# brianz98/A-Fortran-Electronic-Structure-Program

Measured on AMD Instinct MI355X. Metric: CCSD iter wall-time (s) + (T) wall-time (s); fp64 TFLOP/s vs MFMA peak, higher is better.
Workload: dtype f64; 1 GPU; cfg5: nocc=20 nvirt=200, synthetic hashed ERIs scale 0.005; step = 1 CCSD iteration (replicated) + full (T) over i<=j<=k sharded across ranks; nocc=20, nvirt=200, triples=1540, parallelism=(T) ijk-shard x1, CCSD replicas

## Files before the change

### a-fortran-electronic-structure-program_amd/csrc/afesp_internal.h

```cpp
#pragma once
#include <hip/hip_runtime.h>
#include <stdint.h>

#include <map>
#include <stdexcept>
#include <string>
#include <thread>
#include <vector>

#include "gett.h"
#include "tgemm.h"

namespace afesp {

struct Error : std::runtime_error {
    int code;
    Error(int c, const std::string& m) : std::runtime_error(m), code(c) {}
};

#define AFESP_HIP(expr)                                                                                    \
    do {                                                                                                   \
        hipError_t e_ = (expr);                                                                            \
        if (e_ != hipSuccess)                                                                              \
            throw ::afesp::Error(2, std::string(#expr) + ": " + hipGetErrorString(e_) + " (" + __FILE__ + \
// ... 121 lines not shown
    int64_t lam_clock = 0;
    const void* lt_ops_owner = nullptr;
    int64_t lt_ops_stamp = -1, lt_ops_scratch = -1;
    Tensor tensor(std::initializer_list<int64_t> dims);
    void sync();
    void quiesce();
    ~Context();
};

Tensor view(double* d, std::initializer_list<int64_t> dims);

void contract(Context& cx, double alpha, const Tensor& A, const char* la, const Tensor& B, const char* lb, double beta,
              const Tensor& C, const char* lc, int nbatch = 1, const int64_t* bA = nullptr, const int64_t* bB = nullptr,
              const int64_t* bC = nullptr, int force_split = 0, int force_tm = 0, int force_tn = 0);

struct ContractCall {
    double alpha;
    const Tensor* A;
    const char* la;
    const Tensor* B;
    const char* lb;
    double beta;
    const Tensor* C;
    const char* lc;
};
void contract_pair(Context& cx, const ContractCall& c1, const ContractCall& c2);

void permute_add(Context& cx, double alpha, const Tensor& in, const char* li, double beta, const Tensor& out,
                 const char* lo);

void k_fill(Context& cx, double* x, int64_t n, double val);
void k_copy(Context& cx, double* dst, const double* src, int64_t n);
void k_axpby(Context& cx, double* y, double a, const double* x, double b, int64_t n);
void k_ivv_diag(Context& cx, double* ivv, const double* y, const double* x, int o, int v, int a0, int a1);
void k_div(Context& cx, double* out, const double* num, const double* den, int64_t n);
void k_antisym_pair(Context& cx, double* out, const double* in, int64_t d0, int64_t d1, int64_t d2, int64_t d3,
                    int which);
void k_asym_c(Context& cx, double* asym, double* c, const double* t1, const double* t2, int o, int v);
void k_t2_update(Context& cx, double* t2, const double* r2, const double* r2b, const double* r2c, const double* v_oovv, const double* D2,
                 const double* pp, int o, int v, double* t1, const double* r1, const double* r1b, const double* D1, const double* r2y = nullptr);
void k_add_swapped(Context& cx, double* out, const double* y, int o, int v);
void k_r2_full(Context& cx, double* out, const double* r2, const double* pp, int o, int v);
void k_denominators(Context& cx, double* D1, double* D2, const double* e, int o, int v);
void k_vvvv_sympack_packed(Context& cx, double* vs, double* va, const double* packed, int o, int v, int64_t ks, int64_t ka);
void k_c_sympack(Context& cx, double* cs, double* ca, const double* c, int o, int v, int64_t ns, int64_t na, bool half = false);
void k_oooo_pair_expand_add(Context& cx, double* I, const double* xs, const double* xa, int o, int64_t ns, int64_t na);
void k_oooo_sympack(Context& cx, double* is, double* ia, const double* I, int o, int64_t ns, int64_t na);
void k_rows_append(Context& cx, double* dst, int64_t ld, int64_t k0, const double* src, int64_t ns, int64_t ncol);
void k_pp_expand(Context& cx, double* pp, const double* ps, const double* pa, int o, int v, int64_t ns, int64_t na,
                 int64_t p0 = 0, int64_t p1 = -1);
void k_vvx_sympack(Context& cx, double* ws, double* wa, const double* x, int v, int64_t ncol, int64_t ks, int64_t ka);
void k_pair_expand_add(Context& cx, double* out, const double* ps, const double* pa, int o, int64_t ncol, int64_t ns, int64_t na);
void k_ooov_r1_trace(Context& cx, double* r1x, const double* ps, const double* pa, int o, int v, int64_t ns, int64_t na);
void k_cc_energy(Context& cx, double* out2, const double* v_oovv, const double* t1, const double* t2, double* t2_old,
                 int o, int v);
void k_final_sum(Context& cx, double* out, int nq, bool accumulate);
void k_lincomb(Context& cx, double* out, const double* xbase, int64_t xstride, const double* coef_dev, int nx,
               int64_t n);
void k_diis_solve(Context& cx, double* coef, double* bmat, double* flag, int n, int nerr, int slot);
void k_diis_push(Context& cx, double* ht, double* he, const double* amp, const double* amp_s, const double* hist_e, int64_t stride, int ny,
                 int slot, int64_t n);
struct CCTail {
    double *t2, *t1;
    const double *r2, *r1, *voovv, *D2, *D1, *pp;
    double* t2_old;
    int o, v;
// ... 30 lines not shown
```

### a-fortran-electronic-structure-program_amd/csrc/ccsd.h

```cpp
#pragma once
#include "afesp_internal.h"

namespace afesp {

struct DiisRing {
    int nerr = 0, nact = 0, it = 0;
    int64_t nvec = 0;
    double *amp = nullptr;
    double *amp_s = nullptr;
    double *hist_t = nullptr, *hist_e = nullptr;
    double *coef = nullptr;
    double *bmat = nullptr;
    bool tail_pending = false;
    int tail_slot = 0, tail_n = 0;
    double tail_b[256];
};
void diis_alloc(Context& cx, DiisRing& r, int diis_nerr);
void diis_save(Context& cx, DiisRing& r);
void diis_update(Context& cx, DiisRing& r);

struct CCState : DiisRing {
    int o = 0, v = 0;
    bool ready = false;
    double* e = nullptr;
// ... 6 lines not shown
    int sh_rank = 0, sh_world = 1;
    int64_t* pp_tab = nullptr;
    bool pp_sym = false;
    double *pp_vs = nullptr, *pp_va = nullptr, *pp_cs = nullptr, *pp_ca = nullptr, *pp_ps = nullptr, *pp_pa = nullptr;
    int64_t pp_ks = 0, pp_ka = 0, pp_ns = 0, pp_na = 0, pp_kn = 0;
    int64_t pp_lds = 0, pp_lda = 0;
    double *pp_ts = nullptr, *pp_ta = nullptr;
    double *oo_vs = nullptr, *oo_va = nullptr;
    double *oo_xs = nullptr, *oo_xa = nullptr;
    bool cs_packed = false;
    double* r1x = nullptr;
    bool r1x_valid = false;
    int hist_plain = 0;
    bool amps_touched = true;
    int64_t pp_nm = 0;
    double *ov_ws = nullptr, *ov_wa = nullptr;
    Tensor I_vo, I_vv, I_oo_p, I_oo, c, asym, x_voov, I_oooo, I_ovov, I_voov, I_ooov_p;
    Tensor z_ooov;
    double energy = 0.0, energy_old = 0.0, rms = 0.0;
    void* tplan = nullptr;
    Tensor I_vovv_pp, I_ooov_pp;
    const double* eri_src = nullptr;
    double* eri_own = nullptr;
    bool have_cr = false;
    int64_t amp_epoch = 0, cr_epoch = 0;
    void* ring = nullptr;
    bool partials_live = false;
    int64_t frozen_id = 0;
};
void triples_plan_free(CCState& s);

bool ring_tg_applies(const CCState& s);
bool ring_tg_pack(Context& cx, CCState& s);
void ring_tg_intermediates(Context& cx, CCState& s);
void ring_tg_residual(Context& cx, CCState& s);
void ring_tg_materialize(Context& cx, CCState& s, const Tensor& I_ovov_out, const Tensor& I_voov_out);
bool ring_live(const CCState& s);
bool ring_res_live(const CCState& s);
void ring_res_clear(CCState& s);
void ring_invalidate(CCState& s);
void ring_reinit(CCState& s);
const double* ring_Y(const CCState& s);
void ring_free(Context& cx, CCState& s);

void ccsd_init(Context& cx, CCState& s, int o, int v, const double* eri_mo_dev, const double* e_host, int diis_nerr);
bool ccsd_can_reinit(const CCState& s, int o, int v, int diis_nerr);
void ccsd_need_vvvv(Context& cx, CCState& s);
void ccsd_refresh_sharding(Context& cx, CCState& s);
bool ccsd_uses_lanes(const CCState& s);
void ccsd_diis_save(Context& cx, CCState& s);
void ccsd_intermediates(Context& cx, CCState& s, bool save_for_diis = false);
void ccsd_amplitudes(Context& cx, CCState& s, bool defer_update = false);
void ccsd_tail_launch(Context& cx, CCState& s);
int ccsd_tail_read(Context& cx, CCState& s, double e_tol, double t_tol);
void ccsd_pp_ladder(Context& cx, CCState& s);
void ccsd_ooov_pair_form(Context& cx, CCState& s, double* out = nullptr, int64_t a0 = 0, int64_t a1 = 0);
const double* ccsd_residual_full(Context& cx, CCState& s, bool r2);
void ccsd_build_I_vovv_p(Context& cx, CCState& s, const Tensor& out);
bool pp_sym_pays(int64_t o, int64_t v);
int ccsd_energy(Context& cx, CCState& s, double e_tol, double t_tol);
void ccsd_energy_launch(Context& cx, CCState& s);
int ccsd_energy_read(Context& cx, CCState& s, double e_tol, double t_tol);
void ccsd_diis_update(Context& cx, CCState& s);
void ccsd_free(Context& cx, CCState& s);

int64_t triples_count(int o);
void triples_shard_bounds(int o, int v, bool cr, int world, int64_t* bounds);
int triples_block_size(int o, int v, bool cr);
// ... 6 lines not shown
```

### a-fortran-electronic-structure-program_amd/csrc/ccsd.hip

```cpp
#include <algorithm>
#include <cmath>
#include <cstdlib>
#include <cstring>

#include "ccsd.h"
#include "comm.h"
#include "fused.h"

namespace afesp {

static inline int64_t tri64(int64_t i, int64_t j) { return i >= j ? i * (i + 1) / 2 + j : j * (j + 1) / 2 + i; }

bool ccsd_can_reinit(const CCState& s, int o, int v, int diis_nerr)
{
    if (!knobs().cc_reinit) return false;
    return s.ready && s.o == o && s.v == v && s.nerr == diis_nerr && s.pp_sym == pp_sym_pays(o, v);
}

void ccsd_init(Context& cx, CCState& s, int o, int v, const double* eri_mo_dev, const double* e_host, int diis_nerr)
{
    if (o <= 0 || v <= 0) throw Error(1, "ccsd_init: need at least one occupied and one virtual orbital");
    const bool again = ccsd_can_reinit(s, o, v, diis_nerr);
    if (again) {
        cx.quiesce();
// ... 243 lines not shown
    } else {
        k_copy(cx, s.I_oo.d, s.I_oo_p.d, s.I_oo.size());
    }
    C(1.0, s.t1, "je", s.I_vo, "ei", 1.0, s.I_oo, "ji");
    lane(1);
    k_copy(cx, s.I_oooo.d, s.v_oooo.d, s.I_oooo.size());
    if (s.pp_sym && !par && !fused) ccsd_oooo_pair_form(cx, s);
    else C(1.0, s.c, "klef", s.v_oovv, "ijef", 1.0, s.I_oooo, "klij");
    C(1.0, s.t1, "ke", s.v_oovo, "ilej", 1.0, s.I_oooo, "klij");
    C(1.0, s.t1, "le", s.v_oovo, "jkei", 1.0, s.I_oooo, "klij");
    lane(2);
    const int64_t a_len = s.I_ovov.stride[3], a_off = v0 * a_len, a_cnt = (v1 - v0) * a_len;
    if (ivv_diag && s.sharded) {
        if (v1 > v0) C(1.0, s.t1, "je", sl(s.v_vvov, 3), "ebia", 0.0, sl(s.I_ovov, 3), "jbia");
    } else if (ivv_diag) {
        contract_pair(cx, {1.0, &s.t1, "je", &s.v_vvov, "ebia", 0.0, &s.I_ovov, "jbia"}, {1.0, &s.v_vvov, "beia", &s.t1, "je", 0.0, &s.x_voov, "bjia"});
    } else if (v1 > v0) {
        k_copy(cx, s.I_ovov.d + a_off, s.v_ovov.d + a_off, a_cnt);
        if (!ring) C(-0.5, s.v_oovv, "mibe", sl(s.c, 2), "mjae", 1.0, sl(s.I_ovov, 3), "jbia");
        C(-1.0, s.v_oovo, "mibj", sl(s.t1, 1), "ma", 1.0, sl(s.I_ovov, 3), "jbia");
        C(1.0, s.t1, "je", sl(s.v_vvov, 3), "ebia", 1.0, sl(s.I_ovov, 3), "jbia");
    }
    lane(3);
    if (s.sharded) { if (v1 > v0) C(1.0, sl(s.v_vvov, 3), "beia", s.t1, "je", 0.0, sl(s.x_voov, 3), "bjia"); }
    else if (!ivv_diag) C(1.0, s.v_vvov, "beia", s.t1, "je", 0.0, s.x_voov, "bjia");
    if (ivv_diag && v1 > v0) {
        k_ivv_diag(cx, s.I_vv.d, s.I_ovov.d, s.x_voov.d, s.o, s.v, (int)v0, (int)v1);
        k_axpby(cx, s.I_ovov.d + a_off, 1.0, s.v_ovov.d + a_off, 1.0, a_cnt);
        if (!ring) C(-0.5, s.v_oovv, "mibe", sl(s.c, 2), "mjae", 1.0, sl(s.I_ovov, 3), "jbia");
        C(-1.0, s.v_oovo, "mibj", sl(s.t1, 1), "ma", 1.0, sl(s.I_ovov, 3), "jbia");
    }
    const int x_voov_ready = par ? cx.mark() : 0;
    if (v1 > v0) {
        permute_add(cx, 1.0, sl(s.v_oovv, 2), "jiab", 0.0, sl(s.I_voov, 3), "bjia");
        if (fused) C(1.0, s.v_vvov, "beia", s.t1, "je", 1.0, s.I_voov, "bjia");
        else k_axpby(cx, s.I_voov.d + a_off, 1.0, s.x_voov.d + a_off, 1.0, a_cnt);
        if (!ring) {
            C(0.5, s.w_oovv, "imbe", sl(s.t2, 3), "mjea", 1.0, sl(s.I_voov, 3), "bjia");
            C(-0.5, s.v_oovv, "imbe", sl(s.c, 2), "mjae", 1.0, sl(s.I_voov, 3), "bjia");
        }
        C(-1.0, s.v_oovo, "imbj", sl(s.t1, 1), "ma", 1.0, sl(s.I_voov, 3), "bjia");
    }
    if (ring) ring_tg_intermediates(cx, s);
    lane(4);
    if (save_for_diis) diis_save(cx, s);
    if (fused) permute_add(cx, 1.0, s.v_oovo, "kjai", 0.0, s.z_ooov, "jkia");
    C(1.0, s.t1, "ie", s.v_oovv, "mjeb", fused ? 1.0 : 0.0, s.z_ooov, "ijmb");
    C(1.0, s.t1, "je", s.v_ovov, "mbie", 1.0, s.z_ooov, "ijmb");
    lane(5);
    permute_add(cx, 1.0, s.v_oovo, "kjai", 0.0, s.I_ooov_p, "jkia");
    if (s.sharded) {
        Tensor osh = view(cx.scratch("ooov_sh", s.I_ooov_p.size()), {(int64_t)s.o, (int64_t)s.o, (int64_t)s.o, (int64_t)s.v});
        if (v1 > v0) {
            if (s.pp_sym) {
                AFESP_HIP(hipMemsetAsync(osh.d + osh.stride[3] * v0, 0, sizeof(double) * osh.stride[3] * (v1 - v0), cx.stream));
                ccsd_ooov_pair_form(cx, s, osh.d, v0, v1);
            } else {
                C(1.0, s.t2, "jkef", sl(s.v_vvov, 3), "efia", 0.0, sl(osh, 3), "jkia");
            }
            if (par) cx.wait(x_voov_ready);
            C(1.0, s.t1, "je", sl(s.x_voov, 3), "ekia", 1.0, sl(osh, 3), "jkia");
        }
    } else if (s.pp_sym) {
        ccsd_ooov_pair_form(cx, s);
    } else {
        C(1.0, s.t2, "jkef", s.v_vvov, "efia", 1.0, s.I_ooov_p, "jkia");
    }
    if (par) cx.wait(x_voov_ready);
    if (!s.sharded) C(1.0, s.t1, "je", s.x_voov, "ekia", 1.0, s.I_ooov_p, "jkia");
// ... 225 lines not shown
        Tensor r1s = s.r1;
        r1s.d = s.r1_sh;
        C(1.0, s.t1, "ie", slice_axis(s.I_vv, 1, v0, v1), "ea", 1.0, slice_axis(r1s, 1, v0, v1), "ia");
        C(1.0, s.asym, "mief", sl(s.v_vvov, 3), "efma", 1.0, slice_axis(r1s, 1, v0, v1), "ia");
    }
    lane(3);
    if (!sh && !ring) C(1.0, s.asym, "miea", s.I_voov, "ejmb", par ? 0.0 : 1.0, r2c, "ijab");
    if (!open_with_vvov && !sh) C(1.0, s.t1, "ie", s.v_vvov, "baje", 1.0, r2c, "ijab");
    if (!sh) C(-1.0, s.t1, "ma", s.z_ooov, "ijmb", 1.0, r2c, "ijab");
    if (par) cx.join();
    if (sh) {
        const int64_t np = (int64_t)s.v * (s.v + 1) / 2;
        comm_allreduce_dev(cx, cx.comm, s.pp, (int64_t)s.o * s.o * np + s.r2.size() + s.r1.size());
        k_copy(cx, s.r2.d, s.r2_sh, s.r2.size());
        k_axpby(cx, s.r1.d, 1.0, s.r1_sh, 1.0, s.r1.size());
    }
    if (defer_update) return;
    k_t2_update(cx, s.t2.d, s.r2.d, par ? r2b.d : nullptr, par ? r2c.d : nullptr, s.v_oovv.d, s.D2.d, s.pp, s.o, s.v, s.t1.d, s.r1.d,
                par ? r1b.d : nullptr, s.D1.d, ring ? ring_Y(s) : nullptr);
}

const double* ccsd_residual_full(Context& cx, CCState& s, bool r2)
{
    const int64_t n = r2 ? s.r2.size() : s.r1.size();
    double* full = cx.scratch(r2 ? "r2_full" : "r1_full", n);
    auto add_partial = [&](const char* buf) {
        auto it = cx.cache.find(buf);
        if (s.partials_live && it != cx.cache.end()) k_axpby(cx, full, 1.0, (const double*)it->second.first, 1.0, n);
    };
    if (r2) {
        k_r2_full(cx, full, s.r2.d, s.pp, s.o, s.v);
        add_partial(R2_LANE2);
        add_partial(R2_LANE3);
        if (ring_res_live(s)) k_add_swapped(cx, full, ring_Y(s), s.o, s.v);
    } else {
        k_copy(cx, full, s.r1.d, n);
        add_partial(R1_LANE5);
    }
    return full;
}

void ccsd_build_I_vovv_p(Context& cx, CCState& s, const Tensor& out)
{
    permute_add(cx, 1.0, s.v_vvov, "baic", 0.0, out, "ciab");
    contract(cx, -1.0, s.v_oovv, "micb", s.t1, "ma", 1.0, out, "ciab");
    contract(cx, -1.0, s.v_ovov, "maic", s.t1, "mb", 1.0, out, "ciab");
}

void ccsd_tail_launch(Context& cx, CCState& s)
{
    auto launch = [](Context& c, CCState* st) {
        CCTail a;
        a.t2 = st->t2.d; a.t1 = st->t1.d; a.r2 = st->r2.d; a.r1 = st->r1.d; a.voovv = st->v_oovv.d; a.D2 = st->D2.d; a.D1 = st->D1.d;
        a.pp = st->pp; a.t2_old = st->t2_old.d; a.o = st->o; a.v = st->v;
        a.r2y = ring_res_live(*st) ? ring_Y(*st) : nullptr;
        a.half_hist = st->hist_plain == 0;
        if (st->hist_plain > 0) --st->hist_plain;
        a.nerr = st->nerr;
        a.ny = 0; a.slot = 0;
        a.ht = a.he = nullptr; a.amp_s = a.hist_e = nullptr; a.stride = st->nvec;
        a.coef = st->coef; a.bmat = st->bmat;
        if (st->nerr >= 2) {
            int it = st->it + 1;
            if (it > st->nerr) it -= st->nerr;
            a.slot = it - 1;
            a.ny = std::min(st->nact + 1, st->nerr);
            a.ht = st->hist_t + (int64_t)a.slot * st->nvec;
// ... 180 lines not shown
```

### a-fortran-electronic-structure-program_amd/csrc/kernels.hip

```cpp
#include "device_util.h"
#include "fused.h"

namespace afesp {

namespace {
__global__ void fill_kernel(double* x, int64_t n, double val) { GRID_STRIDE(i, n) x[i] = val; }
__global__ void axpby_kernel(double* y, double a, const double* x, double b, int64_t n)
{
    GRID_STRIDE(i, n) y[i] = a * x[i] + (b != 0.0 ? b * y[i] : 0.0);
}
__global__ void div_kernel(double* out, const double* num, const double* den, int64_t n) { GRID_STRIDE(i, n) out[i] = num[i] / den[i]; }

__global__ void antisym_pair_kernel(double* out, const double* in, int64_t d0, int64_t d1, int64_t d2, int64_t d3, int which)
{
    const int64_t n = d0 * d1 * d2 * d3;
    GRID_STRIDE(x, n)
    {
        int64_t i0 = x % d0, r = x / d0, i1 = r % d1;
        r /= d1;
        int64_t i2 = r % d2, i3 = r / d2;
        int64_t y = which == 0 ? i1 + d0 * (i0 + d1 * (i2 + d2 * i3)) : i0 + d0 * (i1 + d1 * (i3 + d2 * i2));
        out[x] = 2.0 * in[x] - in[y];
    }
}

__global__ void asym_c_kernel(double* asym, double* c, const double* t1, const double* t2, int o, int v)
{
    const int64_t n = (int64_t)o * o * v * v;
    GRID_STRIDE(x, n)
    {
        int i = (int)(x % o);
        int64_t r = x / o;
        int j = (int)(r % o);
        r /= o;
        int a = (int)(r % v), b = (int)(r / v);
        double t = t2[x];
        asym[x] = 2.0 * t - t2[j + (int64_t)o * (i + (int64_t)o * (a + (int64_t)v * b))];
        c[x] = t + t1[i + o * a] * t1[j + o * b];
    }
}

__global__ void t2_update_kernel(double* t2, const double* r2, const double* r2b, const double* r2c, const double* voovv, const double* D2,
                                 const double* pp, int o, int v, double* t1, const double* r1, const double* r1b, const double* D1,
                                 const double* r2y)
{
    const int64_t n = (int64_t)o * o * v * v, n1 = (int64_t)o * v;
    GRID_STRIDE(x, n)
    {
        int i = (int)(x % o);
        int64_t r = x / o;
        int j = (int)(r % o);
        r /= o;
        int a = (int)(r % v), b = (int)(r / v);
        int64_t y = j + (int64_t)o * (i + (int64_t)o * (b + (int64_t)v * a));
        const int64_t lad = (a <= b) ? i + (int64_t)o * (j + (int64_t)o * ((int64_t)b * (b + 1) / 2 + a))
                                     : j + (int64_t)o * (i + (int64_t)o * ((int64_t)a * (a + 1) / 2 + b));
        double rx = r2[x], ry = r2[y];
        if (r2b) { rx += r2b[x]; ry += r2b[y]; }
        if (r2c) { rx += r2c[x]; ry += r2c[y]; }
        if (r2y) {
            rx += r2y[j + (int64_t)o * (i + (int64_t)o * (a + (int64_t)v * b))];
            ry += r2y[i + (int64_t)o * (j + (int64_t)o * (b + (int64_t)v * a))];
        }
        t2[x] = (rx + ry + pp[lad] + voovv[x]) / D2[x];
        if (x < n1) t1[x] = (r1[x] + (r1b ? r1b[x] : 0.0)) / D1[x];
    }
}

__global__ void denominators_kernel(double* D1, double* D2, const double* e, int o, int v)
{
    const int64_t n = (int64_t)o * o * v * v;
    GRID_STRIDE(x, n)
    {
        int i = (int)(x % o);
        int64_t r = x / o;
        int j = (int)(r % o);
        r /= o;
        int a = (int)(r % v), b = (int)(r / v);
        D2[x] = e[i] + e[j] - e[a + o] - e[b + o];
        if (j == 0 && b == 0) D1[i + o * a] = e[i] - e[a + o];
    }
}

__global__ __launch_bounds__(TB) void cc_energy_kernel(double* partial, const double* voovv, const double* t1, const double* t2,
                                                       double* t2_old, int o, int v)
{
    __shared__ double sm[8];
    const int64_t n = (int64_t)o * o * v * v;
    double acc[2] = {0.0, 0.0};
    GRID_STRIDE(x, n)
    {
        int i = (int)(x % o);
        int64_t r = x / o;
        int j = (int)(r % o);
        r /= o;
// ... 69 lines not shown
}

void preload_kernels()
{
    first_use_touch(reinterpret_cast<const void*>(fill_kernel));
    (void)hipGetLastError();
}

void k_fill(Context& cx, double* x, int64_t n, double val)
{
    if (cx.rec) {
        if (n > 0) cx.rec->opaque({}, {frange(x, n)}, [=](Context& c_) { k_fill(c_, x, n, val); });
        return;
    }
    if (n > 0) LAUNCH(fill_kernel, dim3(grid_for(n)), x, n, val);
}
void k_copy(Context& cx, double* dst, const double* src, int64_t n)
{
    if (cx.rec) {
        const int64_t one = 1;
        if (n > 0) cx.rec->elementwise(dst, src, 1, &n, &one, &one, 1.0, 0.0);
        return;
    }
    if (n > 0) AFESP_HIP(hipMemcpyAsync(dst, src, sizeof(double) * n, hipMemcpyDeviceToDevice, cx.stream));
}
void k_axpby(Context& cx, double* y, double a, const double* x, double b, int64_t n)
{
    if (cx.rec) {
        const int64_t one = 1;
        if (n > 0) cx.rec->elementwise(y, x, 1, &n, &one, &one, a, b);
        return;
    }
    if (n > 0) LAUNCH(axpby_kernel, dim3(grid_for(n)), y, a, x, b, n);
}
void k_div(Context& cx, double* out, const double* num, const double* den, int64_t n)
{
    if (cx.rec) {
        if (n > 0) cx.rec->opaque({frange(num, n), frange(den, n)}, {frange(out, n)}, [=](Context& c_) { k_div(c_, out, num, den, n); });
        return;
    }
    if (n > 0) LAUNCH(div_kernel, dim3(grid_for(n)), out, num, den, n);
}
__global__ __launch_bounds__(256) void ivv_diag_kernel(double* ivv, const double* y, const double* x, int o, int v, int a0, int a1)
{
    const int64_t idx0 = (int64_t)blockIdx.x * blockDim.x + threadIdx.x;
    if (idx0 >= (int64_t)v * (a1 - a0)) return;
    const int64_t b = idx0 % v, a = a0 + idx0 / v, idx = b + (int64_t)v * a;
    double sy = 0.0, sx = 0.0;
    for (int m = 0; m < o; ++m) {
        sy += y[m + (int64_t)o * (b + (int64_t)v * (m + (int64_t)o * a))];
        sx += x[b + (int64_t)v * (m + (int64_t)o * (m + (int64_t)o * a))];
    }
    ivv[idx] += 2.0 * sy - sx;
}
void k_ivv_diag(Context& cx, double* ivv, const double* y, const double* x, int o, int v, int a0, int a1)
{
    if (cx.rec) throw Error(2, "k_ivv_diag: not part of a recorded sequence");
    if (a1 > a0) LAUNCH(ivv_diag_kernel, dim3(grid_for((int64_t)v * (a1 - a0))), ivv, y, x, o, v, a0, a1);
}
void k_antisym_pair(Context& cx, double* out, const double* in, int64_t d0, int64_t d1, int64_t d2, int64_t d3, int which)
{
    int64_t n = d0 * d1 * d2 * d3;
    if (n > 0) LAUNCH(antisym_pair_kernel, dim3(grid_for(n)), out, in, d0, d1, d2, d3, which);
}
void k_asym_c(Context& cx, double* asym, double* c, const double* t1, const double* t2, int o, int v)
{
// ... 335 lines not shown
    const double *r2, *r1, *voovv, *D2, *D1, *pp;
    double* t2_old;
    int o, v;
    double *ht, *he;
    const double *amp_s, *hist_e;
    int64_t stride;
    int ny, slot;
    const double* r2y;
    int half;
};
template <int NYT, bool YSW = false>
__global__ __launch_bounds__(TB) void cc_tail_kernel(double* partial, TailArgs p)
{
    __shared__ double sm[18 * 4];
    const int o = p.o, v = p.v, ny = p.ny, slot = p.slot;
    const int64_t n = (int64_t)o * o * v * v, n1 = (int64_t)o * v;
    double acc[18];
#pragma unroll
    for (int j = 0; j < 18; ++j) acc[j] = 0.0;
    const int nyc = ny ? ny - 1 : 0;
    GRID_STRIDE(x, n)
    {
        const int i = (int)(x % o);
        int64_t r = x / o;
        const int j = (int)(r % o);
        r /= o;
        const int a = (int)(r % v), b = (int)(r / v);
        const int64_t y = j + (int64_t)o * (i + (int64_t)o * (b + (int64_t)v * a));
        const int64_t lad = (a <= b) ? i + (int64_t)o * (j + (int64_t)o * ((int64_t)b * (b + 1) / 2 + a))
                                     : j + (int64_t)o * (i + (int64_t)o * ((int64_t)a * (a + 1) / 2 + b));
        double r2x = p.r2[x], r2y = p.r2[y];
        const double ppv = p.pp[lad], vx0 = p.voovv[x], d2 = p.D2[x];
        if (YSW) {
            r2x += p.r2y[j + (int64_t)o * (i + (int64_t)o * (a + (int64_t)v * b))];
            r2y += p.r2y[i + (int64_t)o * (j + (int64_t)o * (b + (int64_t)v * a))];
        }
        const double ria = p.r1[i + o * a], dia = p.D1[i + o * a], rjb = p.r1[j + o * b], djb = p.D1[j + o * b];
        const double vx = p.voovv[i + (int64_t)o * (j + (int64_t)o * (b + (int64_t)v * a))];
        const double told = p.t2_old[x];
        double as2 = 0.0, h[NYT > 0 ? NYT : 1];
        const bool half = YSW && p.half;
        const bool hw = !half || a <= b;
        if (NYT > 0) {
            as2 = p.amp_s[n1 + x];
            if (hw) {
#pragma unroll
                for (int q = 0; q < NYT; ++q) h[q] = p.hist_e[(int64_t)min(q, nyc) * p.stride + n1 + x];
            }
        }
        const double t = (r2x + r2y + ppv + vx0) / d2;
        const double tia = ria / dia, tjb = rjb / djb;
        acc[16] += (2.0 * vx0 - vx) * (t + tia * tjb);
        const double d = t - told;
        acc[17] += d * d;
        p.t2_old[x] = t;
        p.t2[x] = t;
        if (NYT > 0) {
            const double e = t - as2;
            p.ht[n1 + x] = t;
            p.he[n1 + x] = e;
            if (hw) {
                const double ew = (half && a < b) ? 2.0 * e : e;
#pragma unroll
                for (int q = 0; q < NYT; ++q) acc[q] += q < ny ? ew * (q == slot ? e : h[q]) : 0.0;
            }
        }
    }
    GRID_STRIDE(x, n1)
// ... 148 lines not shown
```

### a-fortran-electronic-structure-program_amd/csrc/ring.hip

```cpp
#include <algorithm>
#include <cstdlib>
#include <cstring>

#include "ccsd.h"

namespace afesp {

struct RingTg {
    int64_t ov = 0, Kc = 0, each = 0;
    double* slab = nullptr;
    double *cp, *t2p, *t2x, *asp, *nIo, *Ivo, *F1, *F2, *F3, *Y;
    uint32_t* rc32 = nullptr;
    int64_t *cm1 = nullptr, *cn1 = nullptr, *cm2 = nullptr, *cn2 = nullptr;
    int64_t* tab_block = nullptr;
    TgGroup* groups = nullptr;
    int tiles = 0, mx = 0;
    bool pairs2 = false;
    bool frozen_built = false;
    bool packed = false;
    bool live = false;
    bool res_live = false;
};

__global__ __launch_bounds__(256) void ring_tables_kernel(uint32_t* rc32, int64_t* cm1, int64_t* cn1, int64_t* cm2, int64_t* cn2, int o, int v,
                                                          int64_t Kc)
{
    const int64_t ov = (int64_t)o * v;
    for (int64_t x = (int64_t)blockIdx.x * blockDim.x + threadIdx.x; x < ov + 256; x += (int64_t)gridDim.x * blockDim.x) {
        const int64_t y = x < ov ? x : ov - 1;
        rc32[x] = (uint32_t)(8 * Kc * y);
        if (x < ov + 128) {
            const int64_t p = y % o, q = y / o;
            cm1[x] = Kc * y;
            cn1[x] = y;
            cm2[x] = (int64_t)o * p + (int64_t)o * o * v * q;
            cn2[x] = p + (int64_t)o * o * q;
        }
    }
}

bool ring_tg_applies(const CCState& s)
{
    if (!knobs().ring_tg) return false;
    const int64_t min_ov = knobs().ring_tg_min;
    const int64_t ov = (int64_t)s.o * s.v, Kc = (ov + TG_BK - 1) / TG_BK * TG_BK;
    return !s.sharded && ov >= min_ov && ov >= 2 * TG_BK && 8 * Kc * ov < ((int64_t)1 << 32) - 4096;
}

struct RingPackArgs {
    const double *t1, *t2;
    double *asym, *c, *cp, *t2p, *t2x, *asp;
    int o, v, P, Q;
    int64_t Kc;
    unsigned inv_o, inv_oo;
};
__device__ __forceinline__ unsigned ring_div(unsigned x, unsigned inv) { return inv ? __umulhi(x, inv) : x; }

__global__ __launch_bounds__(256) void ring_pack_kernel(RingPackArgs a)
{
    extern __shared__ double tile[];
    const int o = a.o, v = a.v, oo = o * o, P = a.P, Q = a.Q;
    const int tiles_p = (v + P - 1) / P;
    const int p0 = ((int)blockIdx.x % tiles_p) * P, q0 = ((int)blockIdx.x / tiles_p) * Q;
    const int np = min(P, v - p0), nq = min(Q, v - q0), n = oo * np * nq;
    const unsigned inv_np = np == 1 ? 0u : (unsigned)(((uint64_t)1 << 32) / (unsigned)np + 1);
    const int64_t O = o, V = v;
    for (int idx = threadIdx.x; idx < n; idx += 256) {
        const int r = (int)ring_div((unsigned)idx, a.inv_oo), mj = idx - r * oo;
        const int qq = (int)ring_div((unsigned)r, inv_np), pp = r - qq * np;
        tile[mj + oo * (pp + P * qq)] = a.t2[mj + O * O * ((p0 + pp) + V * (q0 + qq))];
    }
    __syncthreads();
    for (int idx = threadIdx.x; idx < n; idx += 256) {
        const int r = (int)ring_div((unsigned)idx, a.inv_oo), mj = idx - r * oo;
        const int qq = (int)ring_div((unsigned)r, inv_np), pp = r - qq * np;
        const int j = (int)ring_div((unsigned)mj, a.inv_o), m = mj - j * o;
        const int blk = oo * (pp + P * qq);
        const double t = tile[mj + blk], tt = tile[j + o * m + blk];
        const int64_t x = mj + O * O * ((p0 + pp) + V * (q0 + qq));
        a.asym[x] = 2.0 * t - tt;
        a.c[x] = t + a.t1[m + o * (p0 + pp)] * a.t1[j + o * (q0 + qq)];
    }
    for (int idx = threadIdx.x; idx < n; idx += 256) {
        int r = (int)ring_div((unsigned)idx, a.inv_o);
        const int m = idx - r * o;
        int r2 = (int)ring_div((unsigned)r, inv_np);
        const int pp = r - r2 * np;
        const int qq = (int)ring_div((unsigned)r2, a.inv_o), j = r2 - qq * o;
        const int blk = oo * (pp + P * qq);
        const double t = tile[m + o * j + blk], tt = tile[j + o * m + blk];
        const int64_t out = m + O * (p0 + pp) + a.Kc * (j + O * (q0 + qq));
        a.t2p[out] = t;
        a.asp[out] = 2.0 * t - tt;
    }
    const unsigned inv_nq = nq == 1 ? 0u : (unsigned)(((uint64_t)1 << 32) / (unsigned)nq + 1);
    for (int idx = threadIdx.x; idx < n; idx += 256) {
        int r = (int)ring_div((unsigned)idx, a.inv_o);
        const int m = idx - r * o;
        int r2 = (int)ring_div((unsigned)r, inv_nq);
        const int qq = r - r2 * nq;
        const int pp = (int)ring_div((unsigned)r2, a.inv_o), j = r2 - pp * o;
        const double t = tile[m + o * j + oo * (pp + P * qq)];
        const int64_t out = m + O * (q0 + qq) + a.Kc * (j + O * (p0 + pp));
        a.t2x[out] = t;
        a.cp[out] = t + a.t1[m + o * (p0 + pp)] * a.t1[j + o * (q0 + qq)];
    }
}

static RingTg* ring_get(Context& cx, CCState& s)
{
    if (s.ring) return (RingTg*)s.ring;
    RingTg* r = new RingTg();
    s.ring = r;
    const int64_t O = s.o, V = s.v;
    r->ov = O * V;
    r->Kc = (r->ov + TG_BK - 1) / TG_BK * TG_BK;
    r->each = r->Kc * r->ov + 2 * TG_BK;
    r->each = (r->each + 15) / 16 * 16;
    r->slab = cx.alloc(10 * r->each);
    double** bufs[10] = {&r->cp, &r->t2p, &r->t2x, &r->asp, &r->nIo, &r->Ivo, &r->F1, &r->F2, &r->F3, &r->Y};
    for (int q = 0; q < 10; ++q) *bufs[q] = r->slab + q * r->each;
    const int64_t n32 = r->ov + 256, n64 = r->ov + 128;
    int64_t* tab = cx.alloc_i64(4 * n64 + (n32 + 1) / 2 + 8);
    r->cm1 = tab; r->cn1 = tab + n64; r->cm2 = tab + 2 * n64; r->cn2 = tab + 3 * n64;
    r->rc32 = (uint32_t*)(tab + 4 * n64);
    r->tab_block = tab;
    AFESP_KLAUNCH(ring_tables_kernel, dim3((unsigned)std::min<int64_t>((n32 + 255) / 256, 4096)), dim3(256), 0, cx.stream, r->rc32, r->cm1,
                       r->cn1, r->cm2, r->cn2, s.o, s.v, r->Kc);
    AFESP_HIP(hipGetLastError());
    const int M = (int)r->ov, mt = (M + TG_BM - 1) / TG_BM, nt = (M + TG_BN - 1) / TG_BN;
    const int nk1 = (int)(r->Kc / TG_BK), gm = tgemm_group_m(M, nt);
    r->mx = nt;
    r->tiles = 2 * mt * nt;
    auto off = [&](const double* p) { return (int64_t)(p - r->slab); };
    TgGroup g[6] = {};
    auto fill = [&](TgGroup& d, const double* a1, const double* a2, const double* b1, const double* b2, const double* c, const int64_t* cn,
                    int tile0, int nk) {
        d.a1 = off(a1); d.a2 = off(a2); d.b1 = off(b1); d.b2 = off(b2); d.c0 = off(c);
        d.colB = r->rc32; d.offCn = cn;
        d.N = M; d.ntiles = nt; d.tile_start = tile0; d.nk1 = nk1; d.nk = nk;
        d.inv_width = tgemm_inverse(gm * nt);
    };
    fill(g[0], r->t2p, r->cp, r->F2, r->F3, r->Ivo, r->cn1, 0, 2 * nk1);
    fill(g[1], r->cp, r->cp, r->F1, r->F1, r->nIo, r->cn1, mt * nt, nk1);
    g[2].tile_start = 2 * mt * nt;
    fill(g[3], r->t2p, r->Ivo, r->nIo, r->asp, s.r2.d, r->cn2, 0, 2 * nk1);
    fill(g[4], r->nIo, r->nIo, r->t2x, r->t2x, r->Y, r->cn2, mt * nt, nk1);
    g[5].tile_start = 2 * mt * nt;
    r->groups = (TgGroup*)cx.alloc((int64_t)(6 * sizeof(TgGroup) / (sizeof(double)) + 1));
    AFESP_HIP(hipMemcpyAsync(r->groups, g, sizeof(g), hipMemcpyHostToDevice, cx.stream));
    AFESP_HIP(hipStreamSynchronize(cx.stream));
    r->pairs2 = (O % 2 == 0);
    return r;
}

void ring_free(Context& cx, CCState& s)
{
    RingTg* r = (RingTg*)s.ring;
    if (!r) return;
    cx.release(r->slab);
    cx.release(r->tab_block);
    cx.release(r->groups);
    delete r;
    s.ring = nullptr;
}

bool ring_live(const CCState& s) { return s.ring && ((RingTg*)s.ring)->live; }
bool ring_res_live(const CCState& s) { return s.ring && ((RingTg*)s.ring)->res_live; }
void ring_res_clear(CCState& s) { if (s.ring) ((RingTg*)s.ring)->res_live = false; }
const double* ring_Y(const CCState& s) { return ((RingTg*)s.ring)->Y; }

static Tensor kview(const RingTg* r, double* buf, const CCState& s, int pos_m, int pos_p, int pos_x, int pos_e)
{
    Tensor t;
    t.d = buf;
    t.rank = 4;
    const int64_t O = s.o, V = s.v;
    t.dim[pos_m] = O; t.stride[pos_m] = 1;
    t.dim[pos_e] = V; t.stride[pos_e] = O;
    t.dim[pos_p] = O; t.stride[pos_p] = r->Kc;
    t.dim[pos_x] = V; t.stride[pos_x] = r->Kc * O;
    return t;
}

bool ring_tg_pack(Context& cx, CCState& s)
{
    const bool off = !knobs().ring_pack;
    const int64_t oo = (int64_t)s.o * s.o;
    if (off || oo * 8 > 65536 || oo >= 65536 / 4) return false;
    RingTg* r = ring_get(cx, s);
    RingPackArgs a;
    a.t1 = s.t1.d; a.t2 = s.t2.d; a.asym = s.asym.d; a.c = s.c.d;
    a.cp = r->cp; a.t2p = r->t2p; a.t2x = r->t2x; a.asp = r->asp;
    a.o = s.o; a.v = s.v; a.Kc = r->Kc;
    a.P = a.Q = oo * 16 * 8 <= 65536 ? 4 : oo * 4 * 8 <= 65536 ? 2 : 1;
    a.inv_o = tgemm_inverse(s.o);
    a.inv_oo = tgemm_inverse((int)oo);
    const int tiles = ((s.v + a.P - 1) / a.P) * ((s.v + a.Q - 1) / a.Q);
    AFESP_KLAUNCH(ring_pack_kernel, dim3((unsigned)tiles), dim3(256), (size_t)(oo * a.P * a.Q * 8), cx.stream, a);
    AFESP_HIP(hipGetLastError());
    r->packed = true;
    return true;
}

void ring_tg_intermediates(Context& cx, CCState& s)
{
    RingTg* r = ring_get(cx, s);
    if (!r->frozen_built) {
        permute_add(cx, 0.5, s.v_oovv, "mibe", 0.0, kview(r, r->F1, s, 0, 1, 2, 3), "mibe");
        permute_add(cx, 0.5, s.w_oovv, "imbe", 0.0, kview(r, r->F2, s, 1, 0, 2, 3), "imbe");
        permute_add(cx, -0.5, s.v_oovv, "imbe", 0.0, kview(r, r->F3, s, 1, 0, 2, 3), "imbe");
        r->frozen_built = true;
    }
    if (!r->packed) {
        permute_add(cx, 1.0, s.c, "mjae", 0.0, kview(r, r->cp, s, 0, 1, 2, 3), "mjae");
        permute_add(cx, 1.0, s.t2, "mjea", 0.0, kview(r, r->t2p, s, 0, 1, 3, 2), "mjea");
        permute_add(cx, 1.0, s.t2, "mjae", 0.0, kview(r, r->t2x, s, 0, 1, 2, 3), "mjae");
        permute_add(cx, 1.0, s.asym, "miea", 0.0, kview(r, r->asp, s, 0, 1, 3, 2), "miea");
    }
    r->packed = false;
    const int ktail4 = (int)((r->ov - (r->Kc - TG_BK) + 3) / 4);
    TgProblem p{r->slab, r->slab, r->slab, r->rc32, r->cm1, (int)r->ov, true, ktail4};
    p.tag = 1;
    AFESP_HIP(tgemm_launch(p, r->groups, 2, r->tiles, r->mx, cx.stream, cx.tg));
    permute_add(cx, -1.0, s.I_ovov, "jbia", 1.0, kview(r, r->nIo, s, 2, 0, 3, 1), "jbia");
    permute_add(cx, 1.0, s.I_voov, "bjia", 1.0, kview(r, r->Ivo, s, 2, 1, 3, 0), "bjia");
    r->live = true;
}

void ring_tg_residual(Context& cx, CCState& s)
{
    RingTg* r = (RingTg*)s.ring;
    if (!r || !r->live) throw Error(2, "ring_tg_residual: the intermediates of this iteration were not formed on this path");
    const int ktail4 = (int)((r->ov - (r->Kc - TG_BK) + 3) / 4);
    TgProblem p{r->slab, r->slab, r->slab, r->rc32, r->cm2, (int)r->ov, r->pairs2, ktail4};
    p.tag = 1;
    AFESP_HIP(tgemm_launch(p, r->groups + 3, 2, r->tiles, r->mx, cx.stream, cx.tg));
    r->res_live = true;
}

void ring_tg_materialize(Context& cx, CCState& s, const Tensor& I_ovov_out, const Tensor& I_voov_out)
{
    RingTg* r = (RingTg*)s.ring;
    permute_add(cx, -1.0, kview(r, r->nIo, s, 2, 0, 3, 1), "jbia", 0.0, I_ovov_out, "jbia");
    permute_add(cx, 1.0, kview(r, r->Ivo, s, 2, 1, 3, 0), "bjia", 0.0, I_voov_out, "bjia");
}

void ring_reinit(CCState& s)
{
    ring_invalidate(s);
    if (s.ring) ((RingTg*)s.ring)->frozen_built = false;
}

void ring_invalidate(CCState& s)
{
    if (s.ring) { ((RingTg*)s.ring)->live = false; ((RingTg*)s.ring)->res_live = false; ((RingTg*)s.ring)->packed = false; }
}

}
```

### a-fortran-electronic-structure-program_amd/csrc/solver.hip

```cpp
#include <cstdio>
#include <cstring>

#include "solver.h"
#include "integrals.h"

namespace afesp {

void GraphSlot::reset()
{
    if (exec) (void)hipGraphExecDestroy(exec);
    exec = nullptr;
    calls = 0;
    disabled = knobs().no_graph;
}

void Solver::cc_programs_reset(Context& cx)
{
    graph_cc.reset();
    fused_slot_reset(cx, fused_int);
    fused_slot_reset(cx, fused_amp);
    fused_slot_reset(cx, fused_iter);
}

void Solver::destroy(Context& cx)
// ... 229 lines not shown
    if (t->size() > capacity) throw Error(1, std::string("afesp_ccsd_get_tensor: buffer too small for ") + name);
    const double* src = t->d;
    if (t == &vovv) {
        vovv.d = cx.scratch("I_vovv_p", vovv.size());
        ccsd_build_I_vovv_p(cx, s, vovv);
        src = vovv.d;
    } else if (is("r2") || is("r1")) {
        src = ccsd_residual_full(cx, s, is("r2"));
    } else if (ring_live(s) && (is("I_ovov") || is("I_voov"))) {
        Tensor io = view(cx.scratch("ring_I_ovov", t->size()), {O, V, O, V}), iv = view(cx.scratch("ring_I_voov", t->size()), {V, O, O, V});
        ring_tg_materialize(cx, s, io, iv);
        src = is("I_ovov") ? io.d : iv.d;
    }
    AFESP_HIP(hipMemcpyAsync(out, src, sizeof(double) * t->size(), hipMemcpyDeviceToHost, cx.stream));
    cx.sync();
}

double Solver::pp_ladder_flop() const
{
    const double O = cc.o, V = cc.v, ps = V * (V + 1) / 2, pa = V * (V - 1) / 2;
    return cc.pp_sym ? 2.0 * (O * (O + 1) / 2 * ps * ps + O * (O - 1) / 2 * pa * pa) : 2.0 * O * O * V * V * ps;
}

double Solver::iteration_flop() const
{
    const double O = cc.o, V = cc.v, ps = V * (V + 1) / 2, pa = V * (V - 1) / 2, os = O * (O + 1) / 2, oa = O * (O - 1) / 2;
    const bool sym = cc.pp_sym;
    const double pp = pp_ladder_flop();
    const double ooov = sym ? 2.0 * O * V * (os * ps + oa * pa) : 2.0 * O * O * O * V * V * V;
    const double o3v3 = O * O * O * V * V * V;
    const bool large = !ccsd_uses_lanes(cc);
    const double oooo = (sym && large) ? 4.0 * (os * os * ps + oa * oa * pa) : 2.0 * O * O * O * O * V * V;
    const double o2v3 = large ? (sym ? 14.0 : 16.0) : 18.0;
    return pp + ooov + 12.0 * o3v3 + oooo + 2.0 * O * O * O * O * V + o2v3 * O * O * V * V * V + 2.0 * O * V * V * V +
           14.0 * O * O * O * V * V;
}

void Solver::so_init_packed(Context& cx, int nbasis, int nel, const double* host, const double* dev, const double* levels, int diis_nerr,
                            bool foo_as_published)
{
    double* tmp = nullptr;
    if (host) {
        tmp = cx.alloc(neri_of(nbasis));
        AFESP_HIP(hipMemcpyAsync(tmp, host, sizeof(double) * neri_of(nbasis), hipMemcpyHostToDevice, cx.stream));
        dev = tmp;
    }
    cx.drop_scratch("ao2mo_");
    so_programs_reset(cx);
    so_init(cx, so, nbasis, nel, dev, levels, diis_nerr, foo_as_published);
    so.amp_epoch = ++cx.amp_clock;
    if (tmp) cx.release(tmp);
}

void Solver::uso_begin(Context& cx, const Integrals& in, const char* who, const char* hint, int64_t nbasis, int64_t nalpha, int64_t nbeta,
                       bool pointers_ok, int diis_nerr)
{
    if (nbasis <= 0 || nbasis > 512 || nalpha < 0 || nbeta < 0 || nalpha > nbasis || nbeta > nbasis || nalpha + nbeta <= 0 ||
        nalpha + nbeta >= 2 * nbasis || !pointers_ok)
        throw Error(1, std::string(who) + ": bad extents");
    if (!in.uhf_aa || in.uhf_n != nbasis)
        throw Error(1, std::string(who) + ": no UHF MO integrals resident for this basis size (call " + hint + " first)");
    const int64_t o = nalpha + nbeta, v = 2 * nbasis - o;
    cx.drop_scratch("ao2mo_");
    so_programs_reset(cx);
    so_free(cx, so);
    if (!cx.fits(so_state_bytes(o, v, diis_nerr)))
        throw Error(1, std::string(who) + ": the dense spin-orbital state of this system does not fit the free device memory");
// ... 90 lines not shown
```

Baseline: 59.86 TFLOP/s.

## Fold ring-term operands into a combined amplitude and halve ring GEMM depth

The t2 and c ring operands are merged into one packed operand dp = t2 - 0.5*(swapped t2 + t1 t1), so two of the fused ring GEMM groups contract over half the K range. This drops the F3 buffer and adds a precomputed G buffer. The voov intermediate is now built from G, x_voov and a scaled I_ovov. The swapped-residual half-term is folded into the t2 update kernels via an fma. To compensate, two extra generic contractions on nIo are added to the residual assembly. The FLOP model is lowered for this path, so reported throughput only rises if wall time falls more than the counted work.

```diff
diff --git a/a-fortran-electronic-structure-program_amd/csrc/afesp_internal.h b/a-fortran-electronic-structure-program_amd/csrc/afesp_internal.h
--- a/a-fortran-electronic-structure-program_amd/csrc/afesp_internal.h
+++ b/a-fortran-electronic-structure-program_amd/csrc/afesp_internal.h
@@ -177,6 +177,7 @@
 void k_fill(Context& cx, double* x, int64_t n, double val);
 void k_copy(Context& cx, double* dst, const double* src, int64_t n);
 void k_axpby(Context& cx, double* y, double a, const double* x, double b, int64_t n);
+void k_add2(Context& cx, double* y, const double* x1, const double* x2, int64_t n);
 void k_ivv_diag(Context& cx, double* ivv, const double* y, const double* x, int o, int v, int a0, int a1);
 void k_div(Context& cx, double* out, const double* num, const double* den, int64_t n);
 void k_antisym_pair(Context& cx, double* out, const double* in, int64_t d0, int64_t d1, int64_t d2, int64_t d3,
diff --git a/a-fortran-electronic-structure-program_amd/csrc/ccsd.h b/a-fortran-electronic-structure-program_amd/csrc/ccsd.h
--- a/a-fortran-electronic-structure-program_amd/csrc/ccsd.h
+++ b/a-fortran-electronic-structure-program_amd/csrc/ccsd.h
@@ -62,8 +62,10 @@
 
 bool ring_tg_applies(const CCState& s);
 bool ring_tg_pack(Context& cx, CCState& s);
+void ring_tg_open_voov(Context& cx, CCState& s);
 void ring_tg_intermediates(Context& cx, CCState& s);
 void ring_tg_residual(Context& cx, CCState& s);
+void ring_tg_residual_full(Context& cx, CCState& s, double* full);
 void ring_tg_materialize(Context& cx, CCState& s, const Tensor& I_ovov_out, const Tensor& I_voov_out);
 bool ring_live(const CCState& s);
 bool ring_res_live(const CCState& s);
diff --git a/a-fortran-electronic-structure-program_amd/csrc/ccsd.hip b/a-fortran-electronic-structure-program_amd/csrc/ccsd.hip
--- a/a-fortran-electronic-structure-program_amd/csrc/ccsd.hip
+++ b/a-fortran-electronic-structure-program_amd/csrc/ccsd.hip
@@ -299,9 +299,10 @@
     }
     const int x_voov_ready = par ? cx.mark() : 0;
     if (v1 > v0) {
-        permute_add(cx, 1.0, sl(s.v_oovv, 2), "jiab", 0.0, sl(s.I_voov, 3), "bjia");
+        if (ring) ring_tg_open_voov(cx, s);
+        else permute_add(cx, 1.0, sl(s.v_oovv, 2), "jiab", 0.0, sl(s.I_voov, 3), "bjia");
         if (fused) C(1.0, s.v_vvov, "beia", s.t1, "je", 1.0, s.I_voov, "bjia");
-        else k_axpby(cx, s.I_voov.d + a_off, 1.0, s.x_voov.d + a_off, 1.0, a_cnt);
+        else if (!ring) k_axpby(cx, s.I_voov.d + a_off, 1.0, s.x_voov.d + a_off, 1.0, a_cnt);
         if (!ring) {
             C(0.5, s.w_oovv, "imbe", sl(s.t2, 3), "mjea", 1.0, sl(s.I_voov, 3), "bjia");
             C(-0.5, s.v_oovv, "imbe", sl(s.c, 2), "mjae", 1.0, sl(s.I_voov, 3), "bjia");
@@ -593,7 +594,7 @@
         k_r2_full(cx, full, s.r2.d, s.pp, s.o, s.v);
         add_partial(R2_LANE2);
         add_partial(R2_LANE3);
-        if (ring_res_live(s)) k_add_swapped(cx, full, ring_Y(s), s.o, s.v);
+        ring_tg_residual_full(cx, s, full);
     } else {
         k_copy(cx, full, s.r1.d, n);
         add_partial(R1_LANE5);
diff --git a/a-fortran-electronic-structure-program_amd/csrc/kernels.hip b/a-fortran-electronic-structure-program_amd/csrc/kernels.hip
--- a/a-fortran-electronic-structure-program_amd/csrc/kernels.hip
+++ b/a-fortran-electronic-structure-program_amd/csrc/kernels.hip
@@ -9,6 +9,7 @@
 {
     GRID_STRIDE(i, n) y[i] = a * x[i] + (b != 0.0 ? b * y[i] : 0.0);
 }
+__global__ void add2_kernel(double* y, const double* x1, const double* x2, int64_t n) { GRID_STRIDE(i, n) y[i] += x1[i] + x2[i]; }
 __global__ void div_kernel(double* out, const double* num, const double* den, int64_t n) { GRID_STRIDE(i, n) out[i] = num[i] / den[i]; }
 
 __global__ void antisym_pair_kernel(double* out, const double* in, int64_t d0, int64_t d1, int64_t d2, int64_t d3, int which)
@@ -59,8 +60,8 @@
         if (r2b) { rx += r2b[x]; ry += r2b[y]; }
         if (r2c) { rx += r2c[x]; ry += r2c[y]; }
         if (r2y) {
-            rx += r2y[j + (int64_t)o * (i + (int64_t)o * (a + (int64_t)v * b))];
-            ry += r2y[i + (int64_t)o * (j + (int64_t)o * (b + (int64_t)v * a))];
+            rx += fma(0.5, r2y[x], r2y[j + (int64_t)o * (i + (int64_t)o * (a + (int64_t)v * b))]);
+            ry += fma(0.5, r2y[y], r2y[i + (int64_t)o * (j + (int64_t)o * (b + (int64_t)v * a))]);
         }
         t2[x] = (rx + ry + pp[lad] + voovv[x]) / D2[x];
         if (x < n1) t1[x] = (r1[x] + (r1b ? r1b[x] : 0.0)) / D1[x];
@@ -196,6 +197,11 @@
         return;
     }
     if (n > 0) LAUNCH(axpby_kernel, dim3(grid_for(n)), y, a, x, b, n);
+}
+void k_add2(Context& cx, double* y, const double* x1, const double* x2, int64_t n)
+{
+    if (cx.rec) throw Error(2, "k_add2: not part of a recorded sequence");
+    if (n > 0) LAUNCH(add2_kernel, dim3(grid_for(n)), y, x1, x2, n);
 }
 void k_div(Context& cx, double* out, const double* num, const double* den, int64_t n)
 {
@@ -597,8 +603,8 @@
         double r2x = p.r2[x], r2y = p.r2[y];
         const double ppv = p.pp[lad], vx0 = p.voovv[x], d2 = p.D2[x];
         if (YSW) {
-            r2x += p.r2y[j + (int64_t)o * (i + (int64_t)o * (a + (int64_t)v * b))];
-            r2y += p.r2y[i + (int64_t)o * (j + (int64_t)o * (b + (int64_t)v * a))];
+            r2x += fma(0.5, p.r2y[x], p.r2y[j + (int64_t)o * (i + (int64_t)o * (a + (int64_t)v * b))]);
+            r2y += fma(0.5, p.r2y[y], p.r2y[i + (int64_t)o * (j + (int64_t)o * (b + (int64_t)v * a))]);
         }
         const double ria = p.r1[i + o * a], dia = p.D1[i + o * a], rjb = p.r1[j + o * b], djb = p.D1[j + o * b];
         const double vx = p.voovv[i + (int64_t)o * (j + (int64_t)o * (b + (int64_t)v * a))];
diff --git a/a-fortran-electronic-structure-program_amd/csrc/ring.hip b/a-fortran-electronic-structure-program_amd/csrc/ring.hip
--- a/a-fortran-electronic-structure-program_amd/csrc/ring.hip
+++ b/a-fortran-electronic-structure-program_amd/csrc/ring.hip
@@ -9,7 +9,8 @@
 struct RingTg {
     int64_t ov = 0, Kc = 0, each = 0;
     double* slab = nullptr;
-    double *cp, *t2p, *t2x, *asp, *nIo, *Ivo, *F1, *F2, *F3, *Y;
+    double *cp, *dp, *t2x, *asp, *nIo, *Hvo, *F1, *F2, *Y;
+    double* G = nullptr;
     uint32_t* rc32 = nullptr;
     int64_t *cm1 = nullptr, *cn1 = nullptr, *cm2 = nullptr, *cn2 = nullptr;
     int64_t* tab_block = nullptr;
@@ -20,6 +21,7 @@
     bool packed = false;
     bool live = false;
     bool res_live = false;
+    bool res_ops = false;
 };
 
 __global__ __launch_bounds__(256) void ring_tables_kernel(uint32_t* rc32, int64_t* cm1, int64_t* cn1, int64_t* cm2, int64_t* cn2, int o, int v,
@@ -49,7 +51,7 @@
 
 struct RingPackArgs {
     const double *t1, *t2;
-    double *asym, *c, *cp, *t2p, *t2x, *asp;
+    double *asym, *c, *cp, *dp, *t2x, *asp;
     int o, v, P, Q;
     int64_t Kc;
     unsigned inv_o, inv_oo;
@@ -90,7 +92,7 @@
         const int blk = oo * (pp + P * qq);
         const double t = tile[m + o * j + blk], tt = tile[j + o * m + blk];
         const int64_t out = m + O * (p0 + pp) + a.Kc * (j + O * (q0 + qq));
-        a.t2p[out] = t;
+        a.dp[out] = t - 0.5 * (tt + a.t1[m + o * (q0 + qq)] * a.t1[j + o * (p0 + pp)]);
         a.asp[out] = 2.0 * t - tt;
     }
     const unsigned inv_nq = nq == 1 ? 0u : (unsigned)(((uint64_t)1 << 32) / (unsigned)nq + 1);
@@ -117,9 +119,10 @@
     r->Kc = (r->ov + TG_BK - 1) / TG_BK * TG_BK;
     r->each = r->Kc * r->ov + 2 * TG_BK;
     r->each = (r->each + 15) / 16 * 16;
-    r->slab = cx.alloc(10 * r->each);
-    double** bufs[10] = {&r->cp, &r->t2p, &r->t2x, &r->asp, &r->nIo, &r->Ivo, &r->F1, &r->F2, &r->F3, &r->Y};
-    for (int q = 0; q < 10; ++q) *bufs[q] = r->slab + q * r->each;
+    r->slab = cx.alloc(9 * r->each);
+    double** bufs[9] = {&r->cp, &r->dp, &r->t2x, &r->asp, &r->nIo, &r->Hvo, &r->F1, &r->F2, &r->Y};
+    for (int q = 0; q < 9; ++q) *bufs[q] = r->slab + q * r->each;
+    r->G = cx.alloc(O * O * V * V);
     const int64_t n32 = r->ov + 256, n64 = r->ov + 128;
     int64_t* tab = cx.alloc_i64(4 * n64 + (n32 + 1) / 2 + 8);
     r->cm1 = tab; r->cn1 = tab + n64; r->cm2 = tab + 2 * n64; r->cn2 = tab + 3 * n64;
@@ -141,10 +144,10 @@
         d.N = M; d.ntiles = nt; d.tile_start = tile0; d.nk1 = nk1; d.nk = nk;
         d.inv_width = tgemm_inverse(gm * nt);
     };
-    fill(g[0], r->t2p, r->cp, r->F2, r->F3, r->Ivo, r->cn1, 0, 2 * nk1);
+    fill(g[0], r->dp, r->dp, r->F2, r->F2, r->Hvo, r->cn1, 0, nk1);
     fill(g[1], r->cp, r->cp, r->F1, r->F1, r->nIo, r->cn1, mt * nt, nk1);
     g[2].tile_start = 2 * mt * nt;
-    fill(g[3], r->t2p, r->Ivo, r->nIo, r->asp, s.r2.d, r->cn2, 0, 2 * nk1);
+    fill(g[3], r->Hvo, r->Hvo, r->asp, r->asp, s.r2.d, r->cn2, 0, nk1);
     fill(g[4], r->nIo, r->nIo, r->t2x, r->t2x, r->Y, r->cn2, mt * nt, nk1);
     g[5].tile_start = 2 * mt * nt;
     r->groups = (TgGroup*)cx.alloc((int64_t)(6 * sizeof(TgGroup) / (sizeof(double)) + 1));
@@ -159,6 +162,7 @@
     RingTg* r = (RingTg*)s.ring;
     if (!r) return;
     cx.release(r->slab);
+    cx.release(r->G);
     cx.release(r->tab_block);
     cx.release(r->groups);
     delete r;
@@ -191,7 +195,7 @@
     RingTg* r = ring_get(cx, s);
     RingPackArgs a;
     a.t1 = s.t1.d; a.t2 = s.t2.d; a.asym = s.asym.d; a.c = s.c.d;
-    a.cp = r->cp; a.t2p = r->t2p; a.t2x = r->t2x; a.asp = r->asp;
+    a.cp = r->cp; a.dp = r->dp; a.t2x = r->t2x; a.asp = r->asp;
     a.o = s.o; a.v = s.v; a.Kc = r->Kc;
     a.P = a.Q = oo * 16 * 8 <= 65536 ? 4 : oo * 4 * 8 <= 65536 ? 2 : 1;
     a.inv_o = tgemm_inverse(s.o);
@@ -200,31 +204,48 @@
     AFESP_KLAUNCH(ring_pack_kernel, dim3((unsigned)tiles), dim3(256), (size_t)(oo * a.P * a.Q * 8), cx.stream, a);
     AFESP_HIP(hipGetLastError());
     r->packed = true;
+    r->res_ops = false;
     return true;
 }
 
+static void ring_frozen(Context& cx, CCState& s, RingTg* r)
+{
+    if (r->frozen_built) return;
+    permute_add(cx, 0.5, s.v_oovv, "mibe", 0.0, kview(r, r->F1, s, 0, 1, 2, 3), "mibe");
+    permute_add(cx, 0.5, s.w_oovv, "imbe", 0.0, kview(r, r->F2, s, 1, 0, 2, 3), "imbe");
+    Tensor g = s.I_voov;
+    g.d = r->G;
+    permute_add(cx, 1.0, s.v_oovv, "jiab", 0.0, g, "bjia");
+    r->frozen_built = true;
+}
+
+void ring_tg_open_voov(Context& cx, CCState& s)
+{
+    RingTg* r = ring_get(cx, s);
+    ring_frozen(cx, s, r);
+    permute_add(cx, -0.5, s.I_ovov, "jbia", 0.0, s.I_voov, "bjia");
+    k_add2(cx, s.I_voov.d, s.x_voov.d, r->G, s.I_voov.size());
+}
+
 void ring_tg_intermediates(Context& cx, CCState& s)
 {
     RingTg* r = ring_get(cx, s);
-    if (!r->frozen_built) {
-        permute_add(cx, 0.5, s.v_oovv, "mibe", 0.0, kview(r, r->F1, s, 0, 1, 2, 3), "mibe");
-        permute_add(cx, 0.5, s.w_oovv, "imbe", 0.0, kview(r, r->F2, s, 1, 0, 2, 3), "imbe");
-        permute_add(cx, -0.5, s.v_oovv, "imbe", 0.0, kview(r, r->F3, s, 1, 0, 2, 3), "imbe");
-        r->frozen_built = true;
-    }
+    ring_frozen(cx, s, r);
     if (!r->packed) {
         permute_add(cx, 1.0, s.c, "mjae", 0.0, kview(r, r->cp, s, 0, 1, 2, 3), "mjae");
-        permute_add(cx, 1.0, s.t2, "mjea", 0.0, kview(r, r->t2p, s, 0, 1, 3, 2), "mjea");
+        permute_add(cx, 1.0, s.t2, "mjea", 0.0, kview(r, r->dp, s, 0, 1, 3, 2), "mjea");
+        permute_add(cx, -0.5, s.c, "mjae", 1.0, kview(r, r->dp, s, 0, 1, 2, 3), "mjae");
         permute_add(cx, 1.0, s.t2, "mjae", 0.0, kview(r, r->t2x, s, 0, 1, 2, 3), "mjae");
         permute_add(cx, 1.0, s.asym, "miea", 0.0, kview(r, r->asp, s, 0, 1, 3, 2), "miea");
     }
     r->packed = false;
+    r->res_ops = false;
     const int ktail4 = (int)((r->ov - (r->Kc - TG_BK) + 3) / 4);
     TgProblem p{r->slab, r->slab, r->slab, r->rc32, r->cm1, (int)r->ov, true, ktail4};
     p.tag = 1;
     AFESP_HIP(tgemm_launch(p, r->groups, 2, r->tiles, r->mx, cx.stream, cx.tg));
     permute_add(cx, -1.0, s.I_ovov, "jbia", 1.0, kview(r, r->nIo, s, 2, 0, 3, 1), "jbia");
-    permute_add(cx, 1.0, s.I_voov, "bjia", 1.0, kview(r, r->Ivo, s, 2, 1, 3, 0), "bjia");
+    permute_add(cx, 1.0, s.I_voov, "bjia", 1.0, kview(r, r->Hvo, s, 2, 1, 3, 0), "bjia");
     r->live = true;
 }
 
@@ -237,13 +258,27 @@
     p.tag = 1;
     AFESP_HIP(tgemm_launch(p, r->groups + 3, 2, r->tiles, r->mx, cx.stream, cx.tg));
     r->res_live = true;
+    r->res_ops = true;
 }
 
 void ring_tg_materialize(Context& cx, CCState& s, const Tensor& I_ovov_out, const Tensor& I_voov_out)
 {
     RingTg* r = (RingTg*)s.ring;
     permute_add(cx, -1.0, kview(r, r->nIo, s, 2, 0, 3, 1), "jbia", 0.0, I_ovov_out, "jbia");
-    permute_add(cx, 1.0, kview(r, r->Ivo, s, 2, 1, 3, 0), "bjia", 0.0, I_voov_out, "bjia");
+    permute_add(cx, 1.0, kview(r, r->Hvo, s, 2, 1, 3, 0), "bjia", 0.0, I_voov_out, "bjia");
+    permute_add(cx, -0.5, kview(r, r->nIo, s, 2, 1, 3, 0), "bjia", 1.0, I_voov_out, "bjia");
+}
+
+void ring_tg_residual_full(Context& cx, CCState& s, double* full)
+{
+    RingTg* r = (RingTg*)s.ring;
+    if (!r || !r->res_live) return;
+    if (!r->res_ops) throw Error(2, "ring_tg_residual_full: the operands of the last residual's ring terms have been overwritten");
+    k_add_swapped(cx, full, r->Y, s.o, s.v);
+    Tensor out = s.r2;
+    out.d = full;
+    contract(cx, -0.5, kview(r, r->asp, s, 0, 1, 3, 2), "miea", kview(r, r->nIo, s, 2, 0, 3, 1), "jemb", 1.0, out, "ijab");
+    contract(cx, 1.0, kview(r, r->nIo, s, 2, 0, 3, 1), "iema", kview(r, r->t2x, s, 0, 1, 2, 3), "mjeb", 1.0, out, "ijab");
 }
 
 void ring_reinit(CCState& s)
@@ -254,7 +289,10 @@
 
 void ring_invalidate(CCState& s)
 {
-    if (s.ring) { ((RingTg*)s.ring)->live = false; ((RingTg*)s.ring)->res_live = false; ((RingTg*)s.ring)->packed = false; }
-}
-
-}
+    if (s.ring) {
+        RingTg* r = (RingTg*)s.ring;
+        r->live = r->res_live = r->res_ops = r->packed = false;
+    }
+}
+
+}
diff --git a/a-fortran-electronic-structure-program_amd/csrc/solver.hip b/a-fortran-electronic-structure-program_amd/csrc/solver.hip
--- a/a-fortran-electronic-structure-program_amd/csrc/solver.hip
+++ b/a-fortran-electronic-structure-program_amd/csrc/solver.hip
@@ -285,7 +285,8 @@
     const bool large = !ccsd_uses_lanes(cc);
     const double oooo = (sym && large) ? 4.0 * (os * os * ps + oa * oa * pa) : 2.0 * O * O * O * O * V * V;
     const double o2v3 = large ? (sym ? 14.0 : 16.0) : 18.0;
-    return pp + ooov + 12.0 * o3v3 + oooo + 2.0 * O * O * O * O * V + o2v3 * O * O * V * V * V + 2.0 * O * V * V * V +
+    const double ring = large && ring_tg_applies(cc) ? 8.0 : 12.0;
+    return pp + ooov + ring * o3v3 + oooo + 2.0 * O * O * O * O * V + o2v3 * O * O * V * V * V + 2.0 * O * V * V * V +
            14.0 * O * O * O * V * V;
 }
 
```

Result: no change. 59.90 TFLOP/s (median of 2 runs) (+0.1%).
